# nyu-dl/MultimodalGame

Measured on AMD Instinct MI355X. Metric: exchange-steps/sec (whole node), 30-class Adaptive max_exchange=10 bs=64, higher is better.
Workload: dtype f32

## Files before the change

### multimodalgame_amd/csrc/device_utils.h

```cpp
#pragma once
#include <hip/hip_runtime.h>
#include <stdint.h>

namespace mmg {

typedef float f32x4 __attribute__((ext_vector_type(4)));
typedef float f32x2 __attribute__((ext_vector_type(2)));
__device__ __forceinline__ f32x2 pk_fma_clamp(f32x2 a, float k, f32x2 c) {
    f32x2 r;
    const f32x2 k2 = {k, k};
    asm("v_pk_fma_f32 %0, %1, %2, %3 clamp" : "=v"(r) : "v"(a), "v"(k2), "v"(c));
    return r;
}
typedef __attribute__((address_space(1))) const float gfloat;
typedef __attribute__((address_space(1))) const f32x4 gf32x4;
__device__ __forceinline__ gfloat* as_global(const float* p) { return (gfloat*)p; }
typedef __attribute__((address_space(1))) float gfloat_w;
__device__ __forceinline__ gfloat_w* as_global_w(float* p) { return (gfloat_w*)p; }
__device__ __forceinline__ float4 ldg4(gfloat* p) {
    const f32x4 v = *(gf32x4*)p;
    return make_float4(v.x, v.y, v.z, v.w);
}

#define MMG_BLOCK 256
// ... 325 lines not shown
    return make_float2(__builtin_bit_cast(float, (unsigned)u), __builtin_bit_cast(float, (unsigned)(u >> 32)));
}
__device__ __forceinline__ float4 ld_cc4(const float* p) { const float2 a = ld_cc2(p), b = ld_cc2(p + 2); return make_float4(a.x, a.y, b.x, b.y); }

__device__ __forceinline__ void st_ll(float* ll, size_t i, float v, uint32_t epoch) {
    const unsigned long long u = ((unsigned long long)epoch << 32) | (unsigned long long)__builtin_bit_cast(unsigned, v);
    __hip_atomic_store(reinterpret_cast<unsigned long long*>(ll) + i, u, __ATOMIC_RELAXED, __HIP_MEMORY_SCOPE_AGENT);
}
__device__ __forceinline__ void st_ll2(float* ll, size_t i, float v0, float v1, uint32_t epoch) {
    const float e = __builtin_bit_cast(float, epoch);
    st_wt4(ll + 2 * i, make_float4(v0, e, v1, e));
}
__device__ __forceinline__ void st_ll_l2(float* ll, size_t i, float v, uint32_t epoch) {
    const unsigned long long u = ((unsigned long long)epoch << 32) | (unsigned long long)__builtin_bit_cast(unsigned, v);
    __hip_atomic_store(reinterpret_cast<unsigned long long*>(ll) + i, u, __ATOMIC_RELAXED, __HIP_MEMORY_SCOPE_WORKGROUP);
}
__device__ __forceinline__ uint32_t xcc_id() { return __builtin_amdgcn_s_getreg(20 | (0 << 6) | ((4 - 1) << 11)) & 0xfu; }
__device__ __forceinline__ unsigned long long ld_ll(const float* ll, size_t i) {
    return __hip_atomic_load(reinterpret_cast<const unsigned long long*>(ll) + i, __ATOMIC_RELAXED, __HIP_MEMORY_SCOPE_AGENT);
}
__device__ __forceinline__ float ll_value(unsigned long long u) { return __builtin_bit_cast(float, (unsigned)u); }
__device__ __forceinline__ bool ll_fresh(unsigned long long u, uint32_t epoch) { return (uint32_t)(u >> 32) == epoch; }

#define MMG_LL_ERR_BASEHX 6u
__device__ __forceinline__ float4 ll_wait4(const float* ll, size_t i, uint32_t epoch, uint32_t* sync) {
    unsigned long long u0, u1, u2, u3;
    int spins = 0;
    for (;;) {
        u0 = ld_ll(ll, i); u1 = ld_ll(ll, i + 1); u2 = ld_ll(ll, i + 2); u3 = ld_ll(ll, i + 3);
        if (ll_fresh(u0, epoch) && ll_fresh(u1, epoch) && ll_fresh(u2, epoch) && ll_fresh(u3, epoch)) break;
        if (++spins > (1 << 18)) { if (sync) __hip_atomic_store(sync + MMG_SYNC_ERR, MMG_LL_ERR_BASEHX, __ATOMIC_RELAXED, __HIP_MEMORY_SCOPE_AGENT); break; }
    }
    return make_float4(ll_value(u0), ll_value(u1), ll_value(u2), ll_value(u3));
}

__device__ __forceinline__ f32x4 mfma16(float a, float b, f32x4 c) {
    return __builtin_amdgcn_mfma_f32_16x16x4f32(a, b, c, 0, 0, 0);
}

}
```

### multimodalgame_amd/csrc/kernels_bwd.h

```cpp
#pragma once
#include <type_traits>
#include "device_utils.h"
#include "layout.h"

namespace mmg {

template <bool CC = false>
__device__ __forceinline__ float combine_score(const float* part, size_t row, int npb, float b2) {
    float v = 0.f;
    if (npb <= 8) {
        float p[8];
#pragma unroll
        for (int j = 0; j < 8; ++j) p[j] = (j < npb) ? (CC ? __hip_atomic_load(&part[row * npb + j], __ATOMIC_RELAXED, __HIP_MEMORY_SCOPE_AGENT) : part[row * npb + j]) : 0.f;
#pragma unroll
        for (int j = 0; j < 8; ++j) v += p[j];
    } else {
        for (int j = 0; j < npb; ++j) v += part[row * npb + j];
    }
    return v + b2;
}

__host__ __device__ inline size_t partll_at(const Dims& d, int sen_side, size_t row, int npb) { return ((size_t)(sen_side ? 0 : 1) * d.T * d.B + row) * npb; }
__device__ __forceinline__ float combine_score_ll(const Dims& dm, const Tape& tp, int sen_side, size_t row, int npb, float b2, uint32_t epoch, bool need) {
    const size_t at = partll_at(dm, sen_side, row, npb);
// ... 479 lines not shown
    const size_t at = MMG_COEF_BC + (size_t)(2 * agent) * MMG_COEF_REPL + (blockIdx.x & (MMG_COEF_REPL - 1));
    unsigned long long u1, u2;
    for (int spins = 0;; ) {
        u1 = ld_ll(wo.coefll, at); u2 = ld_ll(wo.coefll, at + MMG_COEF_REPL);
        if (ll_fresh(u1, epoch) && ll_fresh(u2, epoch)) break;
        __builtin_amdgcn_s_sleep(2);
        if (++spins > (1 << 20)) { __hip_atomic_store(const_cast<uint32_t*>(sync) + MMG_SYNC_ERR, 10u, __ATOMIC_RELAXED, __HIP_MEMORY_SCOPE_AGENT); return false; }
    }
    bc1 = ll_value(u1); bc2s = ll_value(u2);
    return true;
}
__device__ __forceinline__ float opt_wait_coef(const WgOpt& wo, int agent, uint32_t epoch, const uint32_t* sync) {
    unsigned long long u;
    for (int spins = 0;; ) {
        u = ld_ll(wo.coefll, (size_t)agent * MMG_COEF_REPL + (blockIdx.x & (MMG_COEF_REPL - 1)));
        if (ll_fresh(u, epoch)) break;
        __builtin_amdgcn_s_sleep(2);
        if (++spins > (1 << 20)) { __hip_atomic_store(const_cast<uint32_t*>(sync) + MMG_SYNC_ERR, 10u, __ATOMIC_RELAXED, __HIP_MEMORY_SCOPE_AGENT); return -1.f; }
    }
    return ll_value(u);
}

template <bool OPT>
__global__ __launch_bounds__(MMG_BLOCK) void k_wgrad(const JobTable* __restrict__ jt, const float* __restrict__ x,
                                                     const float* __restrict__ desc, float* __restrict__ part,
                                                     Dims dm, const double* __restrict__ stats, float* __restrict__ losses,
                                                     double* __restrict__ totals, const int* __restrict__ rmap,
                                                     const int* __restrict__ rcount, float* __restrict__ wpart, uint32_t* __restrict__ wcnt,
                                                     const uint32_t* __restrict__ sync, float* __restrict__ grad_tail, WgOpt wo, int gt_stride, WgHead hd
#ifdef MMG_TIMING
                                                     , long long* __restrict__ dbg2
#endif
                                                     ) {
    const int bid = (gt_stride > 0 && (int)blockIdx.x >= gt_stride) ? (int)blockIdx.x - gt_stride + hd.gemm_tiles : (int)blockIdx.x;
    const uint32_t oepoch = OPT ? wo.counter[3] + (uint32_t)wo.oa.bump_mb : 0u;
    const uint32_t ostep = OPT ? wo.counter[1] + 1u : 0u;
    if (OPT && bid > hd.n_wblocks) {
        __shared__ float s_ss[4];
        const int agent = bid - hd.n_wblocks - 1;
        const int n = hd.n_wblocks;
        float ss = 0.f;
        for (int k0 = threadIdx.x; k0 < n; k0 += 8 * MMG_BLOCK) {
            unsigned long long u[8]; bool mine[8], any[8];
#pragma unroll
            for (int q = 0; q < 8; ++q) {
                const int k = k0 + q * MMG_BLOCK;
                mine[q] = (k < n) && ((int)jt->wblock_agent[min(k, n - 1)] == agent);
                any[q] = __any(mine[q]);
                u[q] = 0ull;
            }
            for (int spins = 0;; ) {
                bool fresh = true;
#pragma unroll
                for (int q = 0; q < 8; ++q)
                    if (any[q]) {
                        const unsigned long long v = ld_ll(wo.gnll, (size_t)min(k0 + q * MMG_BLOCK, n - 1));
                        if (mine[q]) { u[q] = v; fresh = fresh && ll_fresh(v, oepoch); }
                    }
                if (!__any(!fresh)) break;
                __builtin_amdgcn_s_sleep(1);
                if (++spins > (1 << 20)) { __hip_atomic_store(const_cast<uint32_t*>(sync) + MMG_SYNC_ERR, 11u, __ATOMIC_RELAXED, __HIP_MEMORY_SCOPE_AGENT); break; }
            }
#pragma unroll
            for (int q = 0; q < 8; ++q) ss += mine[q] ? ll_value(u[q]) : 0.f;
        }
        const float wsum = dpp_wave_sum(ss);
        if ((threadIdx.x & 63) == 0) s_ss[threadIdx.x >> 6] = wsum;
        __syncthreads();
        const uint32_t err = __hip_atomic_load(sync + MMG_SYNC_ERR, __ATOMIC_RELAXED, __HIP_MEMORY_SCOPE_AGENT);
        if (wo.oa.optim_type == MMG_OPT_ADAM && opt_trains(wo.oa, agent) && threadIdx.x < MMG_COEF_REPL) {
            const float astep = (float)(ostep - wo.counter[4 + agent]);
            st_ll(wo.coefll, MMG_COEF_BC + (size_t)(2 * agent) * MMG_COEF_REPL + threadIdx.x, 1.f - powf(0.9f, astep), oepoch);
            st_ll(wo.coefll, MMG_COEF_BC + (size_t)(2 * agent + 1) * MMG_COEF_REPL + threadIdx.x, sqrtf(1.f - powf(0.999f, astep)), oepoch);
        }
        if (threadIdx.x < MMG_COEF_REPL + 1) {
            const float tot = (s_ss[0] + s_ss[1]) + (s_ss[2] + s_ss[3]);
            const float coef = 1.0f / (sqrtf(tot) + 1e-6f);
            if (threadIdx.x < MMG_COEF_REPL) st_ll(wo.coefll, (size_t)agent * MMG_COEF_REPL + threadIdx.x, err != 0u ? -1.f : (coef < 1.f ? coef : 1.f), oepoch);
            else st_ll(wo.coefll, (size_t)4 * MMG_COEF_REPL + agent, tot, oepoch);
        }
        return;
    }
#ifdef MMG_TIMING
    if (threadIdx.x == 0 && blockIdx.x < 4096) dbg2[2 * blockIdx.x] = (long long)wall_clock64();
#define MMG_WG_END() do { __syncthreads(); if (threadIdx.x == 0 && blockIdx.x < 4096) dbg2[2 * blockIdx.x + 1] = (long long)wall_clock64(); } while (0)
#else
#define MMG_WG_END() do {} while (0)
#endif
    constexpr int CH = 64;
    __shared__ __attribute__((aligned(16))) float s_a[2][CH][16];
    __shared__ __attribute__((aligned(16))) float s_b[2][CH][48];
    float (*s_acc)[16][33] = reinterpret_cast<float (*)[16][33]>(&s_b[0][0][0]);
    float* s_part = &s_b[0][0][0];
    __shared__ float s_red[8];
    if (bid == hd.special_block) {
        const ColJob& C = jt->c[hd.special_job];
        float* s_v = &s_b[0][0][0];
        const int Hh = C.ld, Wc = C.cols, nb = C.rows;
        const int p8 = threadIdx.x & 7, jj = threadIdx.x >> 3;
        float wreg[32];
        const bool wfast = (Hh == 256) && (Wc <= 32);
        if (wfast) {
#pragma unroll
            for (int i = 0; i < 32; ++i) wreg[i] = C.wrow[(size_t)(p8 + 8 * i) * Wc + min(jj, Wc - 1)];
        }
        for (int h0 = threadIdx.x; h0 < Hh; h0 += MMG_BLOCK) {
            float a0 = 0.f, a1 = 0.f, a2 = 0.f, a3 = 0.f;
            for (int b0 = 0; b0 < nb; b0 += 64) {
                float v[64];
#pragma unroll
                for (int u = 0; u < 64; ++u) v[u] = C.src[(size_t)min(b0 + u, nb - 1) * Hh + h0];
#pragma unroll
                for (int u = 0; u < 64; u += 4) {
                    a0 += (b0 + u < nb) ? v[u] : 0.f; a1 += (b0 + u + 1 < nb) ? v[u + 1] : 0.f;
                    a2 += (b0 + u + 2 < nb) ? v[u + 2] : 0.f; a3 += (b0 + u + 3 < nb) ? v[u + 3] : 0.f;
                }
            }
            s_v[h0] = (a0 + a1) + (a2 + a3);
        }
        __syncthreads();
        float sq = 0.f;
        for (int j0 = 0; j0 < Wc; j0 += MMG_BLOCK / 8) {
            const int j = j0 + jj;
            float acc = 0.f;
            if (wfast) {
#pragma unroll
                for (int i = 0; i < 32; ++i) acc = fmaf(wreg[i], s_v[p8 + 8 * i], acc);
            } else if (j < Wc) {
                for (int h0 = p8; h0 < Hh; h0 += 8) acc = fmaf(C.wrow[(size_t)h0 * Wc + j], s_v[h0], acc);
            }
            acc = dpp_group_sum<8>(acc);
            if (j < Wc && p8 == 0) { const float gsum = acc * C.scale[j]; C.dst[j] = gsum; sq = fmaf(gsum, gsum, sq); }
        }
        sq = block_sum(sq, s_red);
        if (threadIdx.x == 0) part[bid] = sq;
        if (OPT) {
            if (threadIdx.x == 0) st_ll(wo.gnll, bid, sq, oepoch);
#ifdef MMG_TIMING
        if (threadIdx.x == 0 && bid < 2000) dbg2[8192 + 4 * bid + 2] = (long long)wall_clock64();
#endif
#ifdef MMG_TIMING
            if (threadIdx.x == 0 && bid < 2000) dbg2[8192 + 4 * bid + 2] = (long long)wall_clock64();
#endif
            const int ag = jt->wblock_agent[bid];
            float coef = opt_wait_coef(wo, ag, oepoch, sync), bc1, bc2s;
            if (coef >= 0.f && !opt_wait_bc(wo, ag, oepoch, sync, bc1, bc2s)) coef = -1.f;
            for (int j0 = 0; j0 < Wc && coef >= 0.f; j0 += MMG_BLOCK / 8) {
                const int j = j0 + jj;
                if (j < Wc && p8 == 0) {
                    const int64_t idx = (C.dst - wo.grads) + j;
                    opt_update_one(wo.oa, wo.params, wo.state, idx, C.dst[j], coef, wo.params[idx], wo.state[idx],
                                   wo.oa.optim_type == MMG_OPT_ADAM ? wo.state[wo.oa.total + idx] : 0.f, bc1, bc2s);
                }
            }
        }
        MMG_WG_END();
        return;
    }
    const int lane = threadIdx.x & 63, wave = threadIdx.x >> 6;
    if (bid == hd.n_wblocks) {
        float* s_lc = &s_b[0][0][0];
        LossCoef lc; lc.cw = s_lc; lc.ce = s_lc + 3 * dm.T; lc.cb = s_lc + 6 * dm.T;
        loss_coefficients(dm, stats, lc, losses, totals, !OPT);
        if (threadIdx.x == 0) {
            grad_tail[0] = (__hip_atomic_load(sync + MMG_SYNC_ERR, __ATOMIC_RELAXED, __HIP_MEMORY_SCOPE_AGENT) != 0u) ? 1.f : 0.f;
            grad_tail[1] = (float)stats[stat_glob(dm.T, 0)];
            grad_tail[2] = (float)stats[stat_glob(dm.T, 1)];
            grad_tail[3] = 0.f;
        }
        if (OPT) {
            __shared__ float s_tot[4];
            if (threadIdx.x < 4) {
                unsigned long long u;
                for (int spins = 0;; ) {
                    u = ld_ll(wo.coefll, (size_t)4 * MMG_COEF_REPL + threadIdx.x);
                    if (ll_fresh(u, oepoch)) break;
                    __builtin_amdgcn_s_sleep(2);
                    if (++spins > (1 << 20)) { __hip_atomic_store(const_cast<uint32_t*>(sync) + MMG_SYNC_ERR, 11u, __ATOMIC_RELAXED, __HIP_MEMORY_SCOPE_AGENT); break; }
                }
                s_tot[threadIdx.x] = ll_value(u);
            }
            __syncthreads();
            if (threadIdx.x == 0) {
                bool bad = false;
#pragma unroll
                for (int a = 0; a < 4; ++a) bad = bad || !(s_tot[a] == s_tot[a]) || s_tot[a] > 3.0e38f;
                losses[0] = bad ? __builtin_nanf("") : (float)(-stats[stat_glob(dm.T, 0)] / (double)dm.Bg);
                const uint32_t err = __hip_atomic_load(sync + MMG_SYNC_ERR, __ATOMIC_RELAXED, __HIP_MEMORY_SCOPE_AGENT);
                if (wo.err_host && (err != 0u || *wo.err_host == 0u)) *wo.err_host = err;
                if (err == 0u) {
                    wo.counter[2] = ostep;
#pragma unroll
                    for (int a = 0; a < 4; ++a) if ((wo.oa.trainable >> (4 + a)) & 1) wo.counter[4 + a] += 1u;
                }
                if (wo.oa.bump_mb) { wo.counter[0] += 1u; wo.counter[3] += 1u; }
            }
        }
        return;
    }
    auto tile_of = [&](int vt) {
        const int nwg = hd.gemm_tiles, xq = nwg >> 3, xr = nwg & 7;
        const int xcd = vt & 7, slot = vt >> 3;
        return (xcd < xr ? xcd * (xq + 1) : xr * (xq + 1) + (xcd - xr) * xq) + slot;
    };
    constexpr int MAXMAP = 2048;
    __shared__ unsigned short s_map[MAXMAP];
    const bool use_map = rmap != nullptr;
    const bool is_gemm = bid < hd.gemm_tiles;
    const int tb = dm.T * dm.B;
    const int first_blk = is_gemm ? tile_of(bid) : bid - hd.gemm_tiles;
    const int* const lk = is_gemm ? jt->g_begin : jt->c_begin;
    int begin_l, j0, nact = 0, nact_v = 0;
    int lv[MAXMAP / MMG_BLOCK];
    auto lookup_and_list = [&](auto nl_tag) {
        constexpr int NL = decltype(nl_tag)::value;
        int lkl = lane;
        asm volatile("; job lookup, list variant %1" : "+v"(lkl) : "n"(NL));
        begin_l = lk[lkl];
#pragma unroll
        for (int q = 0; q < NL; ++q) lv[q] = rmap[min((int)threadIdx.x + q * MMG_BLOCK, tb - 1)];
        if (NL > 0) {
            int zl = 0;
            asm volatile("; live-row count: a vector load" : "+v"(zl));
            nact_v = rcount[zl];
        }
        asm volatile("; job lookup landed, %1 list loads in flight" : "+v"(begin_l) : "n"(NL));
        j0 = __popcll(__ballot(begin_l <= first_blk)) - 1;
    };
    const bool short_list = tb <= 3 * MMG_BLOCK;
    if (use_map) {
        if (short_list) lookup_and_list(std::integral_constant<int, 3>{});
        else lookup_and_list(std::integral_constant<int, MAXMAP / MMG_BLOCK>{});
    } else lookup_and_list(std::integral_constant<int, 0>{});
    bool list_pending = use_map;
    auto store_list = [&]() {
        if (!list_pending) return;
        list_pending = false;
        nact = __builtin_amdgcn_readfirstlane(nact_v);
        if (short_list) {
#pragma unroll
            for (int q = 0; q < 3; ++q) s_map[(int)threadIdx.x + q * MMG_BLOCK] = (unsigned short)lv[q];
        } else {
#pragma unroll
            for (int q = 0; q < MAXMAP / MMG_BLOCK; ++q) s_map[(int)threadIdx.x + q * MMG_BLOCK] = (unsigned short)lv[q];
        }
    };
    if (is_gemm) {
      __shared__ int s_arrived;
      for (int vt = bid; vt < hd.gemm_tiles; vt += (gt_stride > 0 ? gt_stride : hd.gemm_tiles)) {
        const int tile = vt == bid ? first_blk : tile_of(vt);
// ... 649 lines not shown
```

### multimodalgame_amd/csrc/kernels_fwd.h

```cpp
#pragma once
#include "device_utils.h"
#include "layout.h"

namespace mmg {

template <bool LLO = false, bool LLA = false>
__device__ __forceinline__ void gemm_nt_tile(int tile, const float* __restrict__ X, int ldx, const float* __restrict__ Wm, int ldw,
                                             const float* __restrict__ bias, float* __restrict__ out, int ldo, int M, int N, int K,
                                             float* ll = nullptr, uint32_t epoch = 0u, uint32_t* sync = nullptr);

#define PREP_CTR_ARRIVE 193
#define PREP_CTR(tp, k) ((tp).pflags + (size_t)(k) * 64)
__host__ __device__ inline size_t prepll_hx(const Dims&) { return 0; }
__host__ __device__ inline size_t prepll_hw0(const Dims& d) { return (size_t)d.B * d.H; }
__host__ __device__ inline size_t prepll_cd(const Dims& d) { return (size_t)d.B * d.H + d.H; }
__host__ __device__ inline size_t prepll_dd(const Dims& d) { return (size_t)d.B * d.H + d.H + (size_t)d.D * d.R; }
#define MMG_REPACK_BLOCKS 8
#define MMG_REPACK_F4 30
__host__ __device__ inline bool prep_has_repack(const Dims& d) { return d.H == 256 && d.W == 32 && d.R == 64; }
template <bool GAME = false>
__device__ __forceinline__ void prep_repack(const Dims& dm, const Params& P, const Tape& tp, const int rb, const uint32_t epoch = 0u) {
    constexpr int H = 256, W = 32, R = 64, NTH = 256;
    const int ldy = R + dm.V;
    for (int idx = rb * NTH + (int)threadIdx.x; idx < MMG_REPACK_F4 * NTH; idx += MMG_REPACK_BLOCKS * NTH) {
        const int j = idx / NTH, t = idx % NTH;
        const int k4 = t >> 2, p4 = t & 3, wv = t >> 6, fi = t & 15, fq = (t & 63) >> 4;
        float v[4];
#pragma unroll
        for (int c = 0; c < 4; ++c) {
            if (j < 12) v[c] = P.p[R_WHH][(size_t)(p4 * 48 + 4 * j + c) * R + k4];
            else if (j < 16) v[c] = P.p[R_Y1_W][(size_t)(p4 * 16 + 4 * (j - 12) + c) * ldy + k4];
            else if (j < 18) v[c] = P.p[R_W_W][(size_t)(4 * (4 * (j - 16) + c) + fq) * R + 16 * wv + fi];
            else if (j < 22) v[c] = P.p[R_WH_W][(size_t)(4 * (4 * (j - 18) + c) + fq) * R + 16 * wv + fi];
            else { const int f = 4 * (j - 22) + c, nt = f >> 3, ks = f & 7; v[c] = P.p[S_BIN_W][(size_t)(4 * ks + fq) * H + 64 * wv + 16 * nt + fi]; }
        }
        if (GAME) st_wt4(tp.wrep + (size_t)idx * 4, make_float4(v[0], v[1], v[2], v[3]));
        else *reinterpret_cast<float4*>(tp.wrep + (size_t)idx * 4) = make_float4(v[0], v[1], v[2], v[3]);
    }
    if (GAME) {
        asm volatile("s_waitcnt vmcnt(0)" ::: "memory");
        __syncthreads();
        if (threadIdx.x == 0) st_ll(tp.gamell, (size_t)dm.B + rb, 1.f, epoch);
    }
    (void)W;
}
template <bool ROLE, bool GAME = false>
__device__ __forceinline__ void prep_body(const Dims& dm, const Params& P, const Tape& tp, const float* __restrict__ desc,
                                          const float* __restrict__ x, const int cpb, const int blk, float* smem, const int bump_mb) {
    const int tid = threadIdx.x;
    const uint32_t epoch = ROLE ? tp.counter[3] + 1u : 0u;
    const int HB = (dm.H + 63) / 64;
    const int nC = (dm.D + cpb - 1) / cpb;
    if (blk >= nC + HB) {
        const int nhx = x ? ((dm.B + 15) / 16) * ((dm.H + 15) / 16) : 0;
        if (blk >= nC + HB + nhx) { prep_repack<GAME>(dm, P, tp, blk - nC - HB - nhx, epoch); return; }
        gemm_nt_tile<ROLE, false>(blk - nC - HB, x, dm.F, P.p[S_IMG_W], dm.F, P.p[S_IMG_B], tp.hx, dm.H, dm.B, dm.H, dm.F, tp.prepll, epoch);
        return;
    }
    if (blk < nC && cpb > 1) {
        const int R = dm.R, V = dm.V, ld = dm.R + dm.V, D = dm.D;
        const int d0 = blk * cpb, nd = min(cpb, D - d0);
        float* s_desc = smem;
        float* s_cd = smem + cpb * V;
        const bool isC = tid < R, isD = tid >= R && tid < 2 * R;
        const int r = isC ? tid : (isD ? tid - R : 0);
        const float* wrow = isD ? P.p[R_WD_W] + (size_t)r * V : P.p[R_Y1_W] + (size_t)r * ld + R;
        float4 wreg[32];
#pragma unroll
        for (int j = 0; j < 32; ++j) wreg[j] = (4 * j < V) ? *reinterpret_cast<const float4*>(wrow + 4 * min(j, V / 4 - 1)) : make_float4(0.f, 0.f, 0.f, 0.f);
        const float by = isC ? P.p[R_Y1_B][r] : 0.f;
        for (int i = tid; i < nd * V; i += blockDim.x) { const float dv = desc[(size_t)d0 * V + i]; s_desc[i] = dv; tp.descc[(size_t)d0 * V + i] = dv; }
        __syncthreads();
        if (isC || isD) {
            for (int c = 0; c < nd; ++c) {
                float a0 = 0.f, a1 = 0.f, a2 = 0.f, a3 = 0.f;
#pragma unroll
                for (int j = 0; j < 32; ++j) {
                    if (4 * j < V) {
                        const float4 dv = *reinterpret_cast<const float4*>(s_desc + c * V + 4 * j);
                        a0 = fmaf(wreg[j].x, dv.x, a0); a1 = fmaf(wreg[j].y, dv.y, a1); a2 = fmaf(wreg[j].z, dv.z, a2); a3 = fmaf(wreg[j].w, dv.w, a3);
                    }
                }
                const float v = (a0 + a1) + (a2 + a3) + by;
                const int d = d0 + c;
                if (isC) { tp.Cd[(size_t)d * R + r] = v; if (ROLE) st_ll(tp.prepll, prepll_cd(dm) + (size_t)d * R + r, v, epoch); tp.CdT[(size_t)r * D + d] = -v; s_cd[c * R + r] = v; if (d < 32) tp.cd32[((size_t)(d >> 2) * R + r) * 4 + (d & 3)] = v; }
                else { tp.Dd[(size_t)d * R + r] = v; if (ROLE) st_ll(tp.prepll, prepll_dd(dm) + (size_t)d * R + r, v, epoch); }
            }
        }
        __syncthreads();
        {
            const int lane = tid & 63, wave = tid >> 6;
            const float w2 = (lane < R) ? P.p[R_Y2_W][lane] : 0.f;
            for (int c = wave; c < nd; c += 4) {
                const float t = dpp_wave_sum((lane < R) ? w2 * s_cd[c * R + lane] : 0.f);
                if (lane == 0) tp.cy[d0 + c] = t + P.p[R_Y2_B][0];
            }
        }
        return;
    }
    if (blk < nC) {
        const int d = blk;
        const int R = dm.R, V = dm.V, ld = dm.R + dm.V;
        float* s_desc = smem;
        for (int v = tid; v < V; v += blockDim.x) { const float dv = desc[(size_t)d * V + v]; s_desc[v] = dv; tp.descc[(size_t)d * V + v] = dv; }
        __syncthreads();
        const float* by1 = P.p[R_Y1_B];
        const bool vec = ((ld & 3) == 0) && ((R & 3) == 0) && ((V & 3) == 0);
        float cy_part = 0.f;
        for (int rr = tid; rr < 2 * R; rr += blockDim.x) {
            if (rr < R) continue;
            const int r = rr - R;
            const float* wrow = P.p[R_WD_W] + (size_t)r * V;
            float a0 = 0.f, a1 = 0.f, a2 = 0.f, a3 = 0.f;
            if ((V & 3) == 0) {
#pragma unroll 8
                for (int v = 0; v < V; v += 4) {
                    const float4 wv = *reinterpret_cast<const float4*>(wrow + v);
                    const float4 dv = *reinterpret_cast<const float4*>(s_desc + v);
                    a0 = fmaf(wv.x, dv.x, a0); a1 = fmaf(wv.y, dv.y, a1); a2 = fmaf(wv.z, dv.z, a2); a3 = fmaf(wv.w, dv.w, a3);
                }
            } else {
                for (int v = 0; v < V; ++v) a0 = fmaf(wrow[v], s_desc[v], a0);
            }
            tp.Dd[(size_t)d * R + r] = (a0 + a1) + (a2 + a3);
            if (ROLE) st_ll(tp.prepll, prepll_dd(dm) + (size_t)d * R + r, (a0 + a1) + (a2 + a3), epoch);
        }
        for (int r = tid; r < R; r += blockDim.x) {
            const float* wrow = P.p[R_Y1_W] + (size_t)r * ld + R;
// ... 39 lines not shown
        const float* bc = P.p[S_CODE_B];
        const int n = (blk - nC) * 64 + (tid >> 2), p4 = tid & 3;
        const int nc = min(n, dm.H - 1);
        const float* wrow = P.p[S_CODE_W] + (size_t)nc * W;
        float a0 = 0.f, a1 = 0.f, a2 = 0.f, a3 = 0.f;
        if ((W & 3) == 0) {
            const int W4 = W >> 2;
            for (int k0 = p4; k0 < W4; k0 += 32) {
                float4 wv[8];
#pragma unroll
                for (int u = 0; u < 8; ++u) wv[u] = *reinterpret_cast<const float4*>(wrow + 4 * min(k0 + 4 * u, W4 - 1));
#pragma unroll
                for (int u = 0; u < 8; ++u) {
                    if (k0 + 4 * u < W4) {
                        const float4 sv = *reinterpret_cast<const float4*>(s_sig + 4 * (k0 + 4 * u));
                        a0 = fmaf(wv[u].x, sv.x, a0); a1 = fmaf(wv[u].y, sv.y, a1); a2 = fmaf(wv[u].z, sv.z, a2); a3 = fmaf(wv[u].w, sv.w, a3);
                    }
                }
            }
        } else {
            for (int k = p4; k < W; k += 4) a0 = fmaf(wrow[k], s_sig[k], a0);
        }
        const float tot = dpp_group_sum<4>((a0 + a1) + (a2 + a3));
        if (p4 == 0 && n < dm.H) { tp.hw0[n] = tot + bc[n]; if (ROLE) st_ll(tp.prepll, prepll_hw0(dm) + n, tot + bc[n], epoch); }
    }
}
__device__ __forceinline__ void prep_consumer_arrive(const Tape& tp) {
    __hip_atomic_fetch_add(PREP_CTR(tp, PREP_CTR_ARRIVE), 1u, __ATOMIC_RELAXED, __HIP_MEMORY_SCOPE_AGENT);
}
__device__ __forceinline__ void prep_closing_role(const Tape& tp, const uint32_t consumers, const int bump_mb) {
    if (threadIdx.x != 0) return;
    int spins = 0;
    while (__hip_atomic_load(PREP_CTR(tp, PREP_CTR_ARRIVE), __ATOMIC_RELAXED, __HIP_MEMORY_SCOPE_AGENT) < consumers) {
        __builtin_amdgcn_s_sleep(8);
        if (++spins > MMG_SPIN_LIMIT) { __hip_atomic_store(tp.sync + MMG_SYNC_ERR, 5u, __ATOMIC_RELAXED, __HIP_MEMORY_SCOPE_AGENT); break; }
    }
    __hip_atomic_store(PREP_CTR(tp, PREP_CTR_ARRIVE), 0u, __ATOMIC_RELAXED, __HIP_MEMORY_SCOPE_AGENT);
    if (bump_mb) tp.counter[0] += 1u;
    tp.counter[3] += 1u;
}
__host__ __device__ inline int prep_blocks(const Dims& d, int cpb, bool with_hx) {
    return (d.D + cpb - 1) / cpb + (d.H + 63) / 64 + (with_hx ? ((d.B + 15) / 16) * ((d.H + 15) / 16) : 0) + (prep_has_repack(d) ? MMG_REPACK_BLOCKS : 0);
}

__global__ __launch_bounds__(MMG_BLOCK) void k_prep(Dims dm, Params P, Tape tp, const float* __restrict__ desc,
                                                    const float* __restrict__ x, int cpb, int bump_mb) {
// ... 614 lines not shown
```

### multimodalgame_amd/csrc/kernels_game.h

```cpp
#pragma once
#include "device_utils.h"
#include "kernels_fast.h"
#include "kernels_fast3.h"
#include "layout.h"

namespace mmg {

#ifdef MMG_TIMING
#define MMG_GT(idx) do { if ((threadIdx.x & 63) == 0) tp.dbg2[(idx)] = (long long)wall_clock64(); } while (0)
#else
#define MMG_GT(idx) do {} while (0)
#endif

struct GameLds {
    typedef Fast3Lds F;
    static constexpr int TMAX = F::TMAX, R = F::R, W = F::W;
    static constexpr int cd = F::total;
    static constexpr int Astep = cd + 32 * R;
    static constexpr int desc = Astep + TMAX * R;
    static constexpr int w2s = desc + 32 * 100;
    static constexpr int total = w2s + 2 * R;
    static constexpr int bwd = F::park;
    static constexpr int coef = bwd;
    static constexpr int dgh = coef + 7 * 64;
// ... 4 lines not shown
    static constexpr int cf = dls + TMAX;
    static constexpr int dhin = cf + 4 * TMAX;
    static constexpr int statv = dhin + TMAX * R;
    static constexpr int sm = statv + 27 * TMAX;
    static constexpr int misc = sm + 32;
    static constexpr int SW = 34, SR = 66;
    static constexpr int sb = misc + 16;
    static constexpr int sg = sb + 4 * TMAX * SW;
    static constexpr int bwd_end = sg + 2 * TMAX * SR;
    static_assert(bwd_end <= F::park + 12 * 256 * 4, "the backward's scratch overlays the W_hh park");
};
__host__ __device__ inline int game_lds_bytes() { return GameLds::total * 4; }

template <int MAXQ>
__device__ __forceinline__ void frag_load_cc(float4 (&f)[MAXQ], const float* __restrict__ row, bool valid, int K, int q) {
#pragma unroll
    for (int j = 0; j < MAXQ; ++j) {
        const int k = q * 4 + 16 * j;
        f[j] = (valid && k < K) ? ld_cc4(row + k) : make_float4(0.f, 0.f, 0.f, 0.f);
    }
}

template <int UB>
__device__ __forceinline__ void game_baseline_role(const Dims& dm, const Params& P, const Tape& tp, int role, int n_roles, uint32_t epoch) {
    __shared__ int s_rid[64 * 16];
    __shared__ int s_nwin;
    __shared__ float s_part[UB][4][16];
    const int B = dm.B, H = dm.H, W = dm.W, R = dm.R, K = dm.K, T = dm.T;
    const int npb = (K + 63) / 64, cpw = npb / UB;
    const int combo = role % (2 * cpw), slot = role / (2 * cpw), nslots = n_roles / (2 * cpw);
    const int which = combo / cpw, byi0 = (combo - which * cpw) * UB;
    const int lane = threadIdx.x & 63, wave = threadIdx.x >> 6;
    const int i = lane & 15, q = lane >> 4;
    const float* W1 = which ? P.p[BS_L1_W] : P.p[BR_L1_W];
    const int ldw = which ? H + W : W + R;
    int n[UB]; bool nv[UB]; float bias[UB], w2[UB];
    float4 w_msg[UB][4], w_st[UB][4];
#pragma unroll
    for (int u = 0; u < UB; ++u) {
        n[u] = ((byi0 + u) * 4 + wave) * 16 + i;
        nv[u] = n[u] < K;
        const float* wrow = W1 + (size_t)(nv[u] ? n[u] : 0) * ldw;
        bias[u] = nv[u] ? (which ? P.p[BS_L1_B][n[u]] : P.p[BR_L1_B][n[u]]) : 0.f;
        w2[u] = nv[u] ? (which ? P.p[BS_L2_W][n[u]] : P.p[BR_L2_W][n[u]]) : 0.f;
        frag_load(w_msg[u], wrow + (which ? H : 0), nv[u], W, q);
        if (!which) frag_load(w_st[u], wrow + W, nv[u], R, q);
    }
    for (int k = threadIdx.x; k < 64 * 16; k += blockDim.x) s_rid[k] = -1;
    __syncthreads();
    if (wave == 0) {
        MMG_GT(3584 + 4 * role);
        const int ts = game_wait_done(tp, B, epoch);
        MMG_GT(3584 + 4 * role + 1);
        int base = 0;
        for (int t = 0; t < T; ++t) {
            const bool act = (lane < B) && (t <= ts);
            const unsigned long long m = __ballot(act);
            const int pos = base + __popcll(m & ((1ull << lane) - 1ull));
            const int w = pos >> 4;
            if (act && (w % nslots) == slot && (w / nslots) < 64) s_rid[(w / nslots) * 16 + (pos & 15)] = t * B + lane;
            base += __popcll(m);
        }
        const int nw = (base + 15) >> 4;
        if (lane == 0) s_nwin = nw > slot ? (nw - slot + nslots - 1) / nslots : 0;
    }
    __syncthreads();
    if (threadIdx.x == 0) { MMG_GT(5120 + 8 * role + 0); }
    const int nwin = s_nwin;
    float* hid = which ? tp.hid_s : tp.hid_r;
    float* part = which ? tp.bs_part : tp.br_part;
    float4 xmA[4], xtA[4], xmB[4], xtB[4];
    unsigned long long ubA[UB][4], ubB[UB][4];
// ... 72 lines not shown
                const float v = (s_part[u][0][rw] + s_part[u][1][rw]) + (s_part[u][2][rw] + s_part[u][3][rw]);
                part[(size_t)rid_w[rw] * npb + byi0 + u] = v;
                st_ll(tp.partll, ((size_t)(which ? 0 : 1) * T * B + (size_t)rid_w[rw]) * npb + byi0 + u, v, epoch);
            }
        }
        __syncthreads();
    };
    if (nwin > 0) request(0, xmA, xtA, ubA);
    for (int kw = 0; kw < nwin; kw += 2) {
        window(kw, xmA, xtA, ubA, xmB, xtB, ubB);
        if (kw + 1 < nwin) window(kw + 1, xmB, xtB, ubB, xmA, xtA, ubA);
    }
    if (threadIdx.x == 0) { MMG_GT(3584 + 4 * role + 2); }
}

struct GameArgs { int n_stats, n_bas, bas_ub; };

template <int D>
__global__ __launch_bounds__(256, 1) void k_game_fast(Dims dm, Params P, Tape tp, ConvArgs ar, GameArgs ga) {
    constexpr int H = 256, W = 32, R = 64, V = 100;
    constexpr int NT = 256, TMAX = Fast3Lds::TMAX;
    static_assert(FastDims<H, W, R, V, D>::ok, "unsupported fast shape");
    extern __shared__ __attribute__((aligned(16))) float lds[];
    const uint32_t epoch = tp.counter[3] + 1u;
    const int bx = (int)blockIdx.x, B = dm.B;
    if (bx >= B) {
        int r = bx - B;
        if (r < ar.nprep) {
            if (threadIdx.x == 0 && r < 256) { MMG_GT(4608 + 2 * r); }
            prep_body<true, true>(dm, P, tp, ar.desc, ar.x, ar.prep_cpb, r, lds, 0);
#ifdef MMG_TIMING
            __syncthreads();
            if (threadIdx.x == 0 && r < 256) { MMG_GT(4608 + 2 * r + 1); }
#endif
            return;
        }
        r -= ar.nprep;
        if (r < ar.nbase) {
            gemm_nt_tile<true, true>(r, tp.prepll, H, P.p[BS_L1_W], H + W, nullptr, tp.basehx, dm.K, B, dm.K, H, tp.basell, epoch, tp.sync);
            return;
        }
        r -= ar.nbase;
        if (r < ga.n_stats) {
            MMG_GT(3072 + 4 * (r * 4 + (int)(threadIdx.x >> 6)));
            stats_pairs<true, true, true, true>(dm, P, tp, 1, r * 4 + (int)(threadIdx.x >> 6), ga.n_stats * 4, epoch);
            MMG_GT(3072 + 4 * (r * 4 + (int)(threadIdx.x >> 6)) + 2);
            return;
        }
        r -= ga.n_stats;
        if (r < ga.n_bas) {
            if (ga.bas_ub == 2) game_baseline_role<2>(dm, P, tp, r, ga.n_bas, epoch);
            else game_baseline_role<1>(dm, P, tp, r, ga.n_bas, epoch);
            return;
        }
        r -= ga.n_bas;
        {
            float* s_c = lds; float* s_p = lds + 256;
            role_wait<8, false>(tp.sync, 1, (uint32_t)B, (uint32_t)dm.D);
            if (r == 0 && threadIdx.x < 64) build_row_map<true>(dm, tp);
            if (threadIdx.x == 0) { MMG_GT(3328 + 2 * r); }
            dC_class<true>(dm, P, tp, r, s_c, s_p);
            if (threadIdx.x == 0) { MMG_GT(3328 + 2 * r + 1); }
        }
        return;
    }
    typedef GameLds G;
    typedef Fast3Lds L;
    float* const s_a = lds + L::a; float* const s_gru = lds + L::gru; float* const s_h = lds + L::h; float* const s_g = lds + L::g;
    float* const s_z = lds + L::z; float* const s_pz = lds + L::pz; float* const s_w = lds + L::w; float* const s_pw = lds + L::pw;
    float* const s_y = lds + L::y; float* const s_pi = lds + L::pi; float* const s_uz = lds + L::uz; float* const s_uw = lds + L::uw;
    float* const s_e = lds + L::e; float* const s_A = lds + L::A; float* const s_gh = lds + L::gh;
    float* const s_us = lds + L::small; float* const s_ps = s_us + 16; float* const s_sb = s_us + 32; float* const s_mask = s_us + 48;
    float* const s_sig = s_us + 80;
    float4* const s_park = reinterpret_cast<float4*>(lds + L::park);
    float* const s_cd = lds + G::cd; float* const s_Astep = lds + G::Astep; float* const s_desc = lds + G::desc; float* const s_w2s = lds + G::w2s;

    const int b = bx, tid = threadIdx.x, lane = tid & 63, wave = tid >> 6;
    const int T = dm.T, Dr = dm.D;
    const bool inject = ar.u_s != nullptr;
    MMG_STAMP(0); if (tid == 0) { MMG_GT(2048 + 16 * b + 0); }
    const uint32_t mb_counter = tp.counter[0] + 1u;
    const uint32_t gb = (uint32_t)(dm.boff + b);
    const int tgt = (int)ar.target[b];
    int t_done = T, w_done = T;
    {
        for (int i = tid; i < L::uz; i += NT) lds[i] = 0.f;
        if (inject) {
            for (int i = tid; i < T * W; i += NT) {
                const int t = i / W, j = i - t * W;
                s_uz[i] = ar.u_z[((size_t)t * B + b) * W + j];
                s_uw[i] = ar.u_w[((size_t)t * B + b) * W + j];
            }
            if (tid < T) s_us[tid] = ar.u_s[(size_t)tid * B + b];
        }
        float wc[W];
#pragma unroll
        for (int j = 0; j < W / 4; ++j) {
            const float4 v = *reinterpret_cast<const float4*>(P.p[S_CODE_W] + (size_t)tid * W + 4 * j);
            wc[4 * j] = v.x; wc[4 * j + 1] = v.y; wc[4 * j + 2] = v.z; wc[4 * j + 3] = v.w;
        }
        const float bc = P.p[S_CODE_B][tid];
        const int m2 = tid >> 3, k2 = tid & 7;
        float wb[32], ww[8];
#pragma unroll
        for (int j = 0; j < 8; ++j) {
            const float4 v = *reinterpret_cast<const float4*>(P.p[S_BIN_W] + (size_t)m2 * H + (j * 8 + k2) * 4);
            wb[4 * j] = v.x; wb[4 * j + 1] = v.y; wb[4 * j + 2] = v.z; wb[4 * j + 3] = v.w;
        }
#pragma unroll
        for (int j = 0; j < 2; ++j) {
            const float4 v = *reinterpret_cast<const float4*>(P.p[R_W_W] + (size_t)m2 * R + k2 * 8 + 4 * j);
            ww[4 * j] = v.x; ww[4 * j + 1] = v.y; ww[4 * j + 2] = v.z; ww[4 * j + 3] = v.w;
        }
        const float bb = P.p[S_BIN_B][m2], bw = P.p[R_W_B][m2];
        const int u3 = tid >> 2, q3 = tid & 3;
        float wih[24];
        float4 whh_tmp[12];
#pragma unroll
        for (int gt = 0; gt < 3; ++gt) {
#pragma unroll
            for (int j = 0; j < 2; ++j) {
                const float4 v = *reinterpret_cast<const float4*>(P.p[R_WIH] + (size_t)(gt * R + u3) * W + q3 * 8 + 4 * j);
                wih[8 * gt + 4 * j] = v.x; wih[8 * gt + 4 * j + 1] = v.y; wih[8 * gt + 4 * j + 2] = v.z; wih[8 * gt + 4 * j + 3] = v.w;
            }
#pragma unroll
            for (int i = 0; i < 4; ++i)
                whh_tmp[gt * 4 + i] = *reinterpret_cast<const float4*>(P.p[R_WHH] + (size_t)(gt * R + u3) * R + q3 * 16 + 4 * i);
        }
        const float b_r = P.p[R_BIH][u3] + P.p[R_BHH][u3], b_u = P.p[R_BIH][R + u3] + P.p[R_BHH][R + u3];
        const float b_in = P.p[R_BIH][2 * R + u3], b_hn = P.p[R_BHH][2 * R + u3];
        const int row4 = tid >> 1, half4 = tid & 1;
        float w4[32];
        {
            const float* src = (row4 < R) ? P.p[R_Y1_W] + (size_t)row4 * (R + V) : P.p[R_WH_W] + (size_t)(row4 - R) * R;
#pragma unroll
            for (int j = 0; j < 8; ++j) {
                const float4 v = *reinterpret_cast<const float4*>(src + (j * 2 + half4) * 4);
                w4[4 * j] = v.x; w4[4 * j + 1] = v.y; w4[4 * j + 2] = v.z; w4[4 * j + 3] = v.w;
            }
        }
        const float b4 = (row4 < R) ? 0.f : P.p[R_WH_B][row4 - R];
        const int d5 = tid >> 3, r5 = tid & 7;
        float ncd[8], w2[8];
        {
            const float4 q0 = *reinterpret_cast<const float4*>(P.p[R_Y2_W] + r5 * 8), q1 = *reinterpret_cast<const float4*>(P.p[R_Y2_W] + r5 * 8 + 4);
            w2[0] = q0.x; w2[1] = q0.y; w2[2] = q0.z; w2[3] = q0.w; w2[4] = q1.x; w2[5] = q1.y; w2[6] = q1.z; w2[7] = q1.w;
        }
        const float4 ws4 = *reinterpret_cast<const float4*>(P.p[R_S_W] + (tid & 15) * 4);
        float dsc[(32 * V + NT - 1) / NT];
#pragma unroll
        for (int k = 0; k < (32 * V + NT - 1) / NT; ++k) { const int i = tid + NT * k; dsc[k] = (i < Dr * V) ? ar.desc[min(i, Dr * V - 1)] : 0.f; }
        const float bs = P.p[R_S_B][0];
        float dd[8];
        if (tid < W) s_sig[tid] = fsigmoid(P.p[S_CODE_BIAS][tid]);
        const size_t i_hw = prepll_hw0(dm) + tid, i_hx = prepll_hx(dm) + (size_t)b * H + tid;
        const size_t i_cd = prepll_cd(dm) + (size_t)min(d5, Dr - 1) * R + r5 * 8, i_dd = prepll_dd(dm) + u3;
        unsigned long long u[18];
        auto load_pairs = [&]() {
            u[0] = ld_ll(tp.prepll, i_hw); u[1] = ld_ll(tp.prepll, i_hx);
#pragma unroll
            for (int k = 0; k < 8; ++k) u[2 + k] = ld_ll(tp.prepll, i_cd + k);
#pragma unroll
            for (int k = 0; k < 8; ++k) u[10 + k] = ld_ll(tp.prepll, i_dd + (size_t)min(q3 * 8 + k, Dr - 1) * R);
        };
        if (!inject) {
            for (int i = tid; i < T * W; i += NT) {
                const int t = i / W, j = i - t * W;
                const uint32_t e = (uint32_t)((t * dm.Bg + gb) * W + j);
                s_uz[i] = philox_uniform(ar.seed, e, mb_counter, 0u);
                s_uw[i] = philox_uniform(ar.seed, e, mb_counter, 2u);
            }
            if (tid < T) s_us[tid] = philox_uniform(ar.seed, (uint32_t)(tid * dm.Bg + gb), mb_counter, 1u);
        }
#pragma unroll
        for (int i = 0; i < 12; ++i) s_park[i * NT + tid] = whh_tmp[i];
#pragma unroll
        for (int k = 0; k < (32 * V + NT - 1) / NT; ++k) { const int i = tid + NT * k; if (i < 32 * V) s_desc[i] = dsc[k]; }
        if (tid == 0) { MMG_GT(2048 + 16 * b + 14); }
        {
            int spins = 0;
            for (;;) {
                load_pairs();
                bool fresh = true;
#pragma unroll
                for (int k = 0; k < 18; ++k) fresh = fresh && ll_fresh(u[k], epoch);
#ifdef MMG_TIMING
                if (tid == 0) tp.dbg2[2048 + 16 * b + 15] = (long long)(spins + 1);
#endif
                if (!__any(!fresh)) break;
                if (++spins > (1 << 16)) { if (lane == 0) __hip_atomic_store(tp.sync + MMG_SYNC_ERR, 5u, __ATOMIC_RELAXED, __HIP_MEMORY_SCOPE_AGENT); break; }
            }
        }
        const float hw0 = ll_value(u[0]), hx = ll_value(u[1]);
#pragma unroll
        for (int k = 0; k < 8; ++k) { ncd[k] = -ll_value(u[2 + k]); dd[k] = (q3 * 8 + k < Dr) ? ll_value(u[10 + k]) : 0.f; }
        float cy5;
        {
            float part = 0.f;
#pragma unroll
            for (int k = 0; k < 8; ++k) part = fmaf(w2[k], -ncd[k], part);
            cy5 = dpp_group_sum<8>(part) + P.p[R_Y2_B][0];
// ... 362 lines not shown
```

Baseline: 130,100.

## Defer counter loads via vector loads and warm kernarg segment in persistent kernels

Counter words such as epoch, step and mb_counter are now read with vector loads issued early and converted to wave-uniform values with readfirstlane only where they are used. This keeps their latency off the critical scalar path at kernel entry. Kernel arguments are prefetched by touching one word per 64-byte line, the LDS zeroing is vectorised, and k_wgrad gets a min-blocks launch bound when OPT is set. The extra vector registers and the occupancy hint could raise register pressure.

```diff
diff --git a/multimodalgame_amd/csrc/device_utils.h b/multimodalgame_amd/csrc/device_utils.h
--- a/multimodalgame_amd/csrc/device_utils.h
+++ b/multimodalgame_amd/csrc/device_utils.h
@@ -371,6 +371,44 @@
 __device__ __forceinline__ float ll_value(unsigned long long u) { return __builtin_bit_cast(float, (unsigned)u); }
 __device__ __forceinline__ bool ll_fresh(unsigned long long u, uint32_t epoch) { return (uint32_t)(u >> 32) == epoch; }
 
+__device__ __forceinline__ uint32_t ld_uniform_v(const uint32_t* p) {
+#ifdef MMG_HEAD_SCALAR_CTR
+    return *p;
+#endif
+    int z = 0;
+    asm volatile("; wave-uniform word: a vector load" : "+v"(z));
+    return p[z];
+}
+__device__ __forceinline__ uint32_t uni(uint32_t v) { return (uint32_t)__builtin_amdgcn_readfirstlane((int)v); }
+#ifdef MMG_HEAD_NO_WARM
+template <int BYTES> struct KernargWarm {};
+template <int BYTES> __device__ __forceinline__ KernargWarm<BYTES> kernarg_request() { return {}; }
+template <int BYTES> __device__ __forceinline__ void kernarg_sink(const KernargWarm<BYTES>&) {}
+#else
+template <int BYTES> struct KernargWarm { uint32_t w[(BYTES + 63) / 64 + 1]; };
+template <int BYTES>
+__device__ __forceinline__ KernargWarm<BYTES> kernarg_request() {
+    typedef __attribute__((address_space(4))) const uint32_t kword;
+    kword* ka = (kword*)__builtin_amdgcn_kernarg_segment_ptr();
+    constexpr int N = (BYTES + 63) / 64;
+    KernargWarm<BYTES> k;
+#pragma unroll
+    for (int i = 0; i < N; ++i) k.w[i] = ka[16 * i];
+    k.w[N] = ka[BYTES / 4 - 1];
+    return k;
+}
+template <int BYTES>
+__device__ __forceinline__ void kernarg_sink(const KernargWarm<BYTES>& k) {
+#pragma unroll
+    for (int i = 0; i < (BYTES + 63) / 64 + 1; ++i) asm volatile("" :: "s"(k.w[i]));
+}
+#endif
+template <class... A> struct KernargBytes;
+template <> struct KernargBytes<> { static constexpr int at(int off) { return off; } };
+template <class T, class... A> struct KernargBytes<T, A...> {
+    static constexpr int at(int off) { return KernargBytes<A...>::at((off + (int)alignof(T) - 1) / (int)alignof(T) * (int)alignof(T) + (int)sizeof(T)); }
+};
+
 #define MMG_LL_ERR_BASEHX 6u
 __device__ __forceinline__ float4 ll_wait4(const float* ll, size_t i, uint32_t epoch, uint32_t* sync) {
     unsigned long long u0, u1, u2, u3;
diff --git a/multimodalgame_amd/csrc/kernels_bwd.h b/multimodalgame_amd/csrc/kernels_bwd.h
--- a/multimodalgame_amd/csrc/kernels_bwd.h
+++ b/multimodalgame_amd/csrc/kernels_bwd.h
@@ -525,7 +525,7 @@
 }
 
 template <bool OPT>
-__global__ __launch_bounds__(MMG_BLOCK) void k_wgrad(const JobTable* __restrict__ jt, const float* __restrict__ x,
+__global__ __launch_bounds__(MMG_BLOCK, OPT ? 4 : 1) void k_wgrad(const JobTable* __restrict__ jt, const float* __restrict__ x,
                                                      const float* __restrict__ desc, float* __restrict__ part,
                                                      Dims dm, const double* __restrict__ stats, float* __restrict__ losses,
                                                      double* __restrict__ totals, const int* __restrict__ rmap,
@@ -535,13 +535,17 @@
                                                      , long long* __restrict__ dbg2
 #endif
                                                      ) {
+    const auto kwarm = kernarg_request<KernargBytes<const JobTable*, const float*, const float*, float*, Dims, const double*, float*, double*, const int*,
+                                                    const int*, float*, uint32_t*, const uint32_t*, float*, WgOpt, int, WgHead>::at(0)>();
     const int bid = (gt_stride > 0 && (int)blockIdx.x >= gt_stride) ? (int)blockIdx.x - gt_stride + hd.gemm_tiles : (int)blockIdx.x;
-    const uint32_t oepoch = OPT ? wo.counter[3] + (uint32_t)wo.oa.bump_mb : 0u;
-    const uint32_t ostep = OPT ? wo.counter[1] + 1u : 0u;
+    kernarg_sink(kwarm);
+    auto epoch_of = [&](uint32_t c3_v) -> uint32_t { return uni(c3_v) + (uint32_t)wo.oa.bump_mb; };
     if (OPT && bid > hd.n_wblocks) {
         __shared__ float s_ss[4];
         const int agent = bid - hd.n_wblocks - 1;
         const int n = hd.n_wblocks;
+        const uint32_t c3_v = ld_uniform_v(wo.counter + 3), c1_v = ld_uniform_v(wo.counter + 1), ca_v = ld_uniform_v(wo.counter + 4 + agent);
+        const uint32_t oepoch = epoch_of(c3_v);
         float ss = 0.f;
         for (int k0 = threadIdx.x; k0 < n; k0 += 8 * MMG_BLOCK) {
             unsigned long long u[8]; bool mine[8], any[8];
@@ -572,7 +576,7 @@
         __syncthreads();
         const uint32_t err = __hip_atomic_load(sync + MMG_SYNC_ERR, __ATOMIC_RELAXED, __HIP_MEMORY_SCOPE_AGENT);
         if (wo.oa.optim_type == MMG_OPT_ADAM && opt_trains(wo.oa, agent) && threadIdx.x < MMG_COEF_REPL) {
-            const float astep = (float)(ostep - wo.counter[4 + agent]);
+            const float astep = (float)(uni(c1_v) + 1u - uni(ca_v));
             st_ll(wo.coefll, MMG_COEF_BC + (size_t)(2 * agent) * MMG_COEF_REPL + threadIdx.x, 1.f - powf(0.9f, astep), oepoch);
             st_ll(wo.coefll, MMG_COEF_BC + (size_t)(2 * agent + 1) * MMG_COEF_REPL + threadIdx.x, sqrtf(1.f - powf(0.999f, astep)), oepoch);
         }
@@ -597,6 +601,7 @@
     float* s_part = &s_b[0][0][0];
     __shared__ float s_red[8];
     if (bid == hd.special_block) {
+        const uint32_t c3_v = OPT ? ld_uniform_v(wo.counter + 3) : 0u;
         const ColJob& C = jt->c[hd.special_job];
         float* s_v = &s_b[0][0][0];
         const int Hh = C.ld, Wc = C.cols, nb = C.rows;
@@ -638,6 +643,7 @@
         sq = block_sum(sq, s_red);
         if (threadIdx.x == 0) part[bid] = sq;
         if (OPT) {
+            const uint32_t oepoch = epoch_of(c3_v);
             if (threadIdx.x == 0) st_ll(wo.gnll, bid, sq, oepoch);
 #ifdef MMG_TIMING
         if (threadIdx.x == 0 && bid < 2000) dbg2[8192 + 4 * bid + 2] = (long long)wall_clock64();
@@ -662,6 +668,7 @@
     }
     const int lane = threadIdx.x & 63, wave = threadIdx.x >> 6;
     if (bid == hd.n_wblocks) {
+        const uint32_t c3_v = OPT ? ld_uniform_v(wo.counter + 3) : 0u, c1_v = OPT ? ld_uniform_v(wo.counter + 1) : 0u;
         float* s_lc = &s_b[0][0][0];
         LossCoef lc; lc.cw = s_lc; lc.ce = s_lc + 3 * dm.T; lc.cb = s_lc + 6 * dm.T;
         loss_coefficients(dm, stats, lc, losses, totals, !OPT);
@@ -673,6 +680,7 @@
         }
         if (OPT) {
             __shared__ float s_tot[4];
+            const uint32_t oepoch = epoch_of(c3_v), ostep = uni(c1_v) + 1u;
             if (threadIdx.x < 4) {
                 unsigned long long u;
                 for (int spins = 0;; ) {
@@ -714,12 +722,14 @@
     const int first_blk = is_gemm ? tile_of(bid) : bid - hd.gemm_tiles;
     const int* const lk = is_gemm ? jt->g_begin : jt->c_begin;
     int begin_l, j0, nact = 0, nact_v = 0;
+    uint32_t oepoch = 0u, c3_v = 0u;
     int lv[MAXMAP / MMG_BLOCK];
     auto lookup_and_list = [&](auto nl_tag) {
         constexpr int NL = decltype(nl_tag)::value;
         int lkl = lane;
         asm volatile("; job lookup, list variant %1" : "+v"(lkl) : "n"(NL));
         begin_l = lk[lkl];
+        if (OPT) c3_v = ld_uniform_v(wo.counter + 3);
 #pragma unroll
         for (int q = 0; q < NL; ++q) lv[q] = rmap[min((int)threadIdx.x + q * MMG_BLOCK, tb - 1)];
         if (NL > 0) {
@@ -729,6 +739,7 @@
         }
         asm volatile("; job lookup landed, %1 list loads in flight" : "+v"(begin_l) : "n"(NL));
         j0 = __popcll(__ballot(begin_l <= first_blk)) - 1;
+        if (OPT) oepoch = epoch_of(c3_v);
     };
     const bool short_list = tb <= 3 * MMG_BLOCK;
     if (use_map) {
diff --git a/multimodalgame_amd/csrc/kernels_fwd.h b/multimodalgame_amd/csrc/kernels_fwd.h
--- a/multimodalgame_amd/csrc/kernels_fwd.h
+++ b/multimodalgame_amd/csrc/kernels_fwd.h
@@ -19,7 +19,7 @@
 #define MMG_REPACK_F4 30
 __host__ __device__ inline bool prep_has_repack(const Dims& d) { return d.H == 256 && d.W == 32 && d.R == 64; }
 template <bool GAME = false>
-__device__ __forceinline__ void prep_repack(const Dims& dm, const Params& P, const Tape& tp, const int rb, const uint32_t epoch = 0u) {
+__device__ __forceinline__ void prep_repack(const Dims& dm, const Params& P, const Tape& tp, const int rb, const uint32_t epoch_v = 0u) {
     constexpr int H = 256, W = 32, R = 64, NTH = 256;
     const int ldy = R + dm.V;
     for (int idx = rb * NTH + (int)threadIdx.x; idx < MMG_REPACK_F4 * NTH; idx += MMG_REPACK_BLOCKS * NTH) {
@@ -40,20 +40,23 @@
     if (GAME) {
         asm volatile("s_waitcnt vmcnt(0)" ::: "memory");
         __syncthreads();
+        const uint32_t epoch = uni(epoch_v) + 1u;
         if (threadIdx.x == 0) st_ll(tp.gamell, (size_t)dm.B + rb, 1.f, epoch);
     }
     (void)W;
 }
 template <bool ROLE, bool GAME = false>
 __device__ __forceinline__ void prep_body(const Dims& dm, const Params& P, const Tape& tp, const float* __restrict__ desc,
-                                          const float* __restrict__ x, const int cpb, const int blk, float* smem, const int bump_mb) {
+                                          const float* __restrict__ x, const int cpb, const int blk, float* smem, const int bump_mb,
+                                          const uint32_t epoch_v = 0u) {
     const int tid = threadIdx.x;
-    const uint32_t epoch = ROLE ? tp.counter[3] + 1u : 0u;
+    uint32_t epoch = (ROLE && !GAME) ? tp.counter[3] + 1u : 0u;
     const int HB = (dm.H + 63) / 64;
     const int nC = (dm.D + cpb - 1) / cpb;
     if (blk >= nC + HB) {
         const int nhx = x ? ((dm.B + 15) / 16) * ((dm.H + 15) / 16) : 0;
-        if (blk >= nC + HB + nhx) { prep_repack<GAME>(dm, P, tp, blk - nC - HB - nhx, epoch); return; }
+        if (blk >= nC + HB + nhx) { prep_repack<GAME>(dm, P, tp, blk - nC - HB - nhx, GAME ? epoch_v : epoch); return; }
+        if (GAME) epoch = uni(epoch_v) + 1u;
         gemm_nt_tile<ROLE, false>(blk - nC - HB, x, dm.F, P.p[S_IMG_W], dm.F, P.p[S_IMG_B], tp.hx, dm.H, dm.B, dm.H, dm.F, tp.prepll, epoch);
         return;
     }
@@ -69,6 +72,7 @@
 #pragma unroll
         for (int j = 0; j < 32; ++j) wreg[j] = (4 * j < V) ? *reinterpret_cast<const float4*>(wrow + 4 * min(j, V / 4 - 1)) : make_float4(0.f, 0.f, 0.f, 0.f);
         const float by = isC ? P.p[R_Y1_B][r] : 0.f;
+        if (GAME) epoch = uni(epoch_v) + 1u;
         for (int i = tid; i < nd * V; i += blockDim.x) { const float dv = desc[(size_t)d0 * V + i]; s_desc[i] = dv; tp.descc[(size_t)d0 * V + i] = dv; }
         __syncthreads();
         if (isC || isD) {
@@ -104,6 +108,7 @@
         float* s_desc = smem;
         for (int v = tid; v < V; v += blockDim.x) { const float dv = desc[(size_t)d * V + v]; s_desc[v] = dv; tp.descc[(size_t)d * V + v] = dv; }
         __syncthreads();
+        if (GAME) epoch = uni(epoch_v) + 1u;
         const float* by1 = P.p[R_Y1_B];
         const bool vec = ((ld & 3) == 0) && ((R & 3) == 0) && ((V & 3) == 0);
         float cy_part = 0.f;
@@ -189,6 +194,7 @@
             for (int k = p4; k < W; k += 4) a0 = fmaf(wrow[k], s_sig[k], a0);
         }
         const float tot = dpp_group_sum<4>((a0 + a1) + (a2 + a3));
+        if (GAME) epoch = uni(epoch_v) + 1u;
         if (p4 == 0 && n < dm.H) { tp.hw0[n] = tot + bc[n]; if (ROLE) st_ll(tp.prepll, prepll_hw0(dm) + n, tot + bc[n], epoch); }
     }
 }
diff --git a/multimodalgame_amd/csrc/kernels_game.h b/multimodalgame_amd/csrc/kernels_game.h
--- a/multimodalgame_amd/csrc/kernels_game.h
+++ b/multimodalgame_amd/csrc/kernels_game.h
@@ -50,7 +50,7 @@
 }
 
 template <int UB>
-__device__ __forceinline__ void game_baseline_role(const Dims& dm, const Params& P, const Tape& tp, int role, int n_roles, uint32_t epoch) {
+__device__ __forceinline__ void game_baseline_role(const Dims& dm, const Params& P, const Tape& tp, int role, int n_roles, uint32_t epoch_v) {
     __shared__ int s_rid[64 * 16];
     __shared__ int s_nwin;
     __shared__ float s_part[UB][4][16];
@@ -76,6 +76,7 @@
     }
     for (int k = threadIdx.x; k < 64 * 16; k += blockDim.x) s_rid[k] = -1;
     __syncthreads();
+    const uint32_t epoch = uni(epoch_v) + 1u;
     if (wave == 0) {
         MMG_GT(3584 + 4 * role);
         const int ts = game_wait_done(tp, B, epoch);
@@ -194,13 +195,16 @@
     constexpr int NT = 256, TMAX = Fast3Lds::TMAX;
     static_assert(FastDims<H, W, R, V, D>::ok, "unsupported fast shape");
     extern __shared__ __attribute__((aligned(16))) float lds[];
-    const uint32_t epoch = tp.counter[3] + 1u;
+    const auto kwarm = kernarg_request<KernargBytes<Dims, Params, Tape, ConvArgs, GameArgs>::at(0)>();
     const int bx = (int)blockIdx.x, B = dm.B;
+    uint32_t* const ctr = tp.counter;
+    kernarg_sink(kwarm);
     if (bx >= B) {
+        const uint32_t epoch_v = ld_uniform_v(ctr + 3);
         int r = bx - B;
         if (r < ar.nprep) {
             if (threadIdx.x == 0 && r < 256) { MMG_GT(4608 + 2 * r); }
-            prep_body<true, true>(dm, P, tp, ar.desc, ar.x, ar.prep_cpb, r, lds, 0);
+            prep_body<true, true>(dm, P, tp, ar.desc, ar.x, ar.prep_cpb, r, lds, 0, epoch_v);
 #ifdef MMG_TIMING
             __syncthreads();
             if (threadIdx.x == 0 && r < 256) { MMG_GT(4608 + 2 * r + 1); }
@@ -209,20 +213,20 @@
         }
         r -= ar.nprep;
         if (r < ar.nbase) {
-            gemm_nt_tile<true, true>(r, tp.prepll, H, P.p[BS_L1_W], H + W, nullptr, tp.basehx, dm.K, B, dm.K, H, tp.basell, epoch, tp.sync);
+            gemm_nt_tile<true, true>(r, tp.prepll, H, P.p[BS_L1_W], H + W, nullptr, tp.basehx, dm.K, B, dm.K, H, tp.basell, uni(epoch_v) + 1u, tp.sync);
             return;
         }
         r -= ar.nbase;
         if (r < ga.n_stats) {
             MMG_GT(3072 + 4 * (r * 4 + (int)(threadIdx.x >> 6)));
-            stats_pairs<true, true, true, true>(dm, P, tp, 1, r * 4 + (int)(threadIdx.x >> 6), ga.n_stats * 4, epoch);
+            stats_pairs<true, true, true, true>(dm, P, tp, 1, r * 4 + (int)(threadIdx.x >> 6), ga.n_stats * 4, uni(epoch_v) + 1u);
             MMG_GT(3072 + 4 * (r * 4 + (int)(threadIdx.x >> 6)) + 2);
             return;
         }
         r -= ga.n_stats;
         if (r < ga.n_bas) {
-            if (ga.bas_ub == 2) game_baseline_role<2>(dm, P, tp, r, ga.n_bas, epoch);
-            else game_baseline_role<1>(dm, P, tp, r, ga.n_bas, epoch);
+            if (ga.bas_ub == 2) game_baseline_role<2>(dm, P, tp, r, ga.n_bas, epoch_v);
+            else game_baseline_role<1>(dm, P, tp, r, ga.n_bas, epoch_v);
             return;
         }
         r -= ga.n_bas;
@@ -251,12 +255,11 @@
     const int T = dm.T, Dr = dm.D;
     const bool inject = ar.u_s != nullptr;
     MMG_STAMP(0); if (tid == 0) { MMG_GT(2048 + 16 * b + 0); }
-    const uint32_t mb_counter = tp.counter[0] + 1u;
     const uint32_t gb = (uint32_t)(dm.boff + b);
-    const int tgt = (int)ar.target[b];
+    uint32_t epoch = 0u;
+    int tgt = 0;
     int t_done = T, w_done = T;
     {
-        for (int i = tid; i < L::uz; i += NT) lds[i] = 0.f;
         if (inject) {
             for (int i = tid; i < T * W; i += NT) {
                 const int t = i / W, j = i - t * W;
@@ -271,6 +274,7 @@
             const float4 v = *reinterpret_cast<const float4*>(P.p[S_CODE_W] + (size_t)tid * W + 4 * j);
             wc[4 * j] = v.x; wc[4 * j + 1] = v.y; wc[4 * j + 2] = v.z; wc[4 * j + 3] = v.w;
         }
+        const uint32_t mbc_v = ld_uniform_v(ctr);
         const float bc = P.p[S_CODE_B][tid];
         const int m2 = tid >> 3, k2 = tid & 7;
         float wb[32], ww[8];
@@ -287,7 +291,7 @@
         const float bb = P.p[S_BIN_B][m2], bw = P.p[R_W_B][m2];
         const int u3 = tid >> 2, q3 = tid & 3;
         float wih[24];
-        float4 whh_tmp[12];
+        f32x4 whh_tmp[12];
 #pragma unroll
         for (int gt = 0; gt < 3; ++gt) {
 #pragma unroll
@@ -297,7 +301,7 @@
             }
 #pragma unroll
             for (int i = 0; i < 4; ++i)
-                whh_tmp[gt * 4 + i] = *reinterpret_cast<const float4*>(P.p[R_WHH] + (size_t)(gt * R + u3) * R + q3 * 16 + 4 * i);
+                whh_tmp[gt * 4 + i] = *reinterpret_cast<const f32x4*>(P.p[R_WHH] + (size_t)(gt * R + u3) * R + q3 * 16 + 4 * i);
         }
         const float b_r = P.p[R_BIH][u3] + P.p[R_BHH][u3], b_u = P.p[R_BIH][R + u3] + P.p[R_BHH][R + u3];
         const float b_in = P.p[R_BIH][2 * R + u3], b_hn = P.p[R_BHH][2 * R + u3];
@@ -335,7 +339,12 @@
 #pragma unroll
             for (int k = 0; k < 8; ++k) u[10 + k] = ld_ll(tp.prepll, i_dd + (size_t)min(q3 * 8 + k, Dr - 1) * R);
         };
+        static_assert(L::uz % 4 == 0, "zeroed as float4");
+#pragma unroll
+        for (int k = 0; k < (L::uz / 4 + NT - 1) / NT; ++k) { const int i = tid + NT * k; if (i < L::uz / 4) reinterpret_cast<float4*>(lds)[i] = make_float4(0.f, 0.f, 0.f, 0.f); }
+        const uint32_t epoch_v = ld_uniform_v(ctr + 3);
         if (!inject) {
+            const uint32_t mb_counter = uni(mbc_v) + 1u;
             for (int i = tid; i < T * W; i += NT) {
                 const int t = i / W, j = i - t * W;
                 const uint32_t e = (uint32_t)((t * dm.Bg + gb) * W + j);
@@ -345,10 +354,12 @@
             if (tid < T) s_us[tid] = philox_uniform(ar.seed, (uint32_t)(tid * dm.Bg + gb), mb_counter, 1u);
         }
 #pragma unroll
-        for (int i = 0; i < 12; ++i) s_park[i * NT + tid] = whh_tmp[i];
+        for (int i = 0; i < 12; ++i) reinterpret_cast<f32x4*>(s_park)[i * NT + tid] = whh_tmp[i];
 #pragma unroll
         for (int k = 0; k < (32 * V + NT - 1) / NT; ++k) { const int i = tid + NT * k; if (i < 32 * V) s_desc[i] = dsc[k]; }
         if (tid == 0) { MMG_GT(2048 + 16 * b + 14); }
+        epoch = uni(epoch_v) + 1u;
+        tgt = (int)ar.target[b];
         {
             int spins = 0;
             for (;;) {
```

Measured after the change: 131,300 (median of 6 runs). Within noise of the previous version (+1.0%).
